# omahs/celestia-app

Measured on AMD Instinct MI355X. Metric: EDS+DAH squares/sec (k=128), higher is better.
Workload: dtype u8; 1 GPU; k=128 ODS -> EDS + 4k NMT roots + DAH, batch replay; k=128, field=GF(2^8), parallelism=batch1, input_layout=ODS in Q0 of the EDS buffer (placed by the upload), batches_in_flight=4

## Files before the change

celestia-app_amd/csrc/nmt_device.hpp:

```cpp
#pragma once
#include <hip/hip_runtime.h>

#include "cel_internal.hpp"
#include "sha256_device.hpp"

namespace cel {

__device__ __forceinline__ void load_node(const uint32_t* p, uint32_t (&n)[kNodeWords]) {
  const uint4* q = reinterpret_cast<const uint4*>(p);
#pragma unroll
  for (int i = 0; i < 6; i++) {
    const uint4 v = q[i];
    n[4 * i] = v.x; n[4 * i + 1] = v.y; n[4 * i + 2] = v.z; n[4 * i + 3] = v.w;
  }
}

__device__ __forceinline__ void store_node(uint32_t* p, const uint32_t (&n)[kNodeWords]) {
  uint4* q = reinterpret_cast<uint4*>(p);
#pragma unroll
  for (int i = 0; i < 6; i++) q[i] = make_uint4(n[4 * i], n[4 * i + 1], n[4 * i + 2], n[4 * i + 3]);
}

__device__ __forceinline__ void put_digest(uint32_t (&nd)[kNodeWords], const uint32_t (&st)[8]) {
  uint32_t sw[8];
#pragma unroll
  for (int i = 0; i < 8; i++) sw[i] = bswap32(st[i]);
  nd[14] = (nd[14] & 0xFFFFu) | (sw[0] << 16);
#pragma unroll
  for (int i = 15; i <= 21; i++) nd[i] = __builtin_amdgcn_alignbyte(sw[i - 14], sw[i - 15], 2);
  nd[22] = sw[7] >> 16;
  nd[23] = 0;
}


constexpr uint32_t kLeafParPrefix[7] = {0x00FFFFFFu, 0xFFFFFFFFu, 0xFFFFFFFFu, 0xFFFFFFFFu,
                                        0xFFFFFFFFu, 0xFFFFFFFFu, 0xFFFFFFFFu};
constexpr ShaMid kLeafParMid = sha_midstate(kLeafParPrefix, 7);

template <bool PF>
__device__ __forceinline__ void leaf_hash(uint32_t (&st)[8], const uint32_t* __restrict__ sh, bool q0) {
  sha256_init(st);
  uint32_t w[16];
  uint32_t nx[17];
  auto load17 = [&](int b) {
    const uint32_t* base = sh + 16 * b - 8;
    const uint4* p4 = reinterpret_cast<const uint4*>(base);
#pragma unroll
    for (int i = 0; i < 4; i++) {
      const uint4 v = p4[i];
      nx[4 * i] = v.x; nx[4 * i + 1] = v.y; nx[4 * i + 2] = v.z; nx[4 * i + 3] = v.w;
    }
    nx[16] = base[16];
  };
  {
    uint32_t s[9];
    const uint4* p4 = reinterpret_cast<const uint4*>(sh);
    const uint4 v0 = p4[0], v1 = p4[1];
    s[0] = v0.x; s[1] = v0.y; s[2] = v0.z; s[3] = v0.w; s[4] = v1.x; s[5] = v1.y; s[6] = v1.z; s[7] = v1.w;
    s[8] = sh[8];
    if (PF) load17(1);
#pragma unroll
    for (int i = 8; i < 16; i++) w[i] = perm(s[i - 8], s[i - 7], 0x06070001u);
    if (__all(!q0)) {
#pragma unroll
      for (int i = 0; i < 7; i++) w[i] = kLeafParPrefix[i];
      w[7] = 0xFFFF0000u | perm(0u, s[0], 0x0C0C0001u);
      sha256_compress_from<7>(st, mid_regs(kLeafParMid), w);
    } else {
      if (q0) {
        w[0] = perm(0u, s[0], 0x0C000102u);
#pragma unroll
        for (int i = 1; i < 7; i++) w[i] = perm(s[i - 1], s[i], 0x07000102u);
        w[7] = perm(s[6], s[7], 0x07000C0Cu) | perm(0u, s[0], 0x0C0C0001u);
      } else {
#pragma unroll
        for (int i = 0; i < 7; i++) w[i] = kLeafParPrefix[i];
        w[7] = 0xFFFF0000u | perm(0u, s[0], 0x0C0C0001u);
      }
      sha256_compress(st, w);
    }
  }
#pragma unroll 1
  for (int b = 1; b < 8; b++) {
    if (!PF) load17(b);
#pragma unroll
    for (int i = 0; i < 16; i++) w[i] = perm(nx[i], nx[i + 1], 0x06070001u);
    if (PF) {
      if (b < 7) {
        load17(b + 1);
      } else {
        const uint4* p4 = reinterpret_cast<const uint4*>(sh + 120);
        const uint4 v0 = p4[0], v1 = p4[1];
        nx[0] = v0.x; nx[1] = v0.y; nx[2] = v0.z; nx[3] = v0.w; nx[4] = v1.x; nx[5] = v1.y; nx[6] = v1.z; nx[7] = v1.w;
      }
    }
    sha256_compress(st, w);
  }
  {
    if (!PF) {
      const uint4* p4 = reinterpret_cast<const uint4*>(sh + 120);
      const uint4 v0 = p4[0], v1 = p4[1];
      nx[0] = v0.x; nx[1] = v0.y; nx[2] = v0.z; nx[3] = v0.w; nx[4] = v1.x; nx[5] = v1.y; nx[6] = v1.z; nx[7] = v1.w;
    }
#pragma unroll
    for (int i = 0; i < 7; i++) w[i] = perm(nx[i], nx[i + 1], 0x06070001u);
    w[7] = perm(nx[7], 0x80u, 0x0607000Cu);
#pragma unroll
    for (int i = 8; i < 15; i++) w[i] = 0u;
    w[15] = 542u * 8u;
    sha256_compress(st, w);
  }
}

__device__ __forceinline__ void leaf_record(const uint32_t* __restrict__ sh, bool q0, const uint32_t (&st)[8],
                                            uint32_t (&nd)[kNodeWords]) {
  if (q0) {
    const uint4* p4 = reinterpret_cast<const uint4*>(sh);
    uint32_t s[8];
    const uint4 v0 = p4[0], v1 = p4[1];
    s[0] = v0.x; s[1] = v0.y; s[2] = v0.z; s[3] = v0.w; s[4] = v1.x; s[5] = v1.y; s[6] = v1.z; s[7] = v1.w;
#pragma unroll
    for (int i = 0; i < 7; i++) nd[i] = s[i];
    nd[7] = (s[7] & 0xFFu) | (s[0] << 8);
#pragma unroll
    for (int i = 0; i < 6; i++) nd[8 + i] = __builtin_amdgcn_alignbyte(s[i + 1], s[i], 3);
    nd[14] = (s[6] >> 24) | ((s[7] & 0xFFu) << 8);
  } else {
#pragma unroll
    for (int i = 0; i < 14; i++) nd[i] = 0xFFFFFFFFu;
    nd[14] = 0xFFFFu;
  }
  put_digest(nd, st);
}

template <bool PF>
__device__ __forceinline__ void make_leaf_node(const uint32_t* __restrict__ sh, bool q0, uint32_t (&nd)[kNodeWords]) {
  uint32_t st[8];
  leaf_hash<PF>(st, sh, q0);
  leaf_record(sh, q0, st, nd);
}

__device__ __forceinline__ bool ns_less(const uint32_t* __restrict__ a, const uint32_t* __restrict__ b) {
  const uint4* pa = reinterpret_cast<const uint4*>(a);
  const uint4* pb = reinterpret_cast<const uint4*>(b);
  uint32_t x[8], y[8];
#pragma unroll
  for (int i = 0; i < 2; i++) {
    const uint4 u = pa[i], v = pb[i];
    x[4 * i] = u.x; x[4 * i + 1] = u.y; x[4 * i + 2] = u.z; x[4 * i + 3] = u.w;
    y[4 * i] = v.x; y[4 * i + 1] = v.y; y[4 * i + 2] = v.z; y[4 * i + 3] = v.w;
  }
  int res = 0;
#pragma unroll
  for (int i = 0; i < 8; i++) {
    uint32_t xa = bswap32(x[i]), yb = bswap32(y[i]);
    if (i == 7) { xa &= 0xFF000000u; yb &= 0xFF000000u; }
    if (res == 0 && xa != yb) res = xa < yb ? -1 : 1;
  }
  return res < 0;
}

__device__ __forceinline__ bool min_is_parity(const uint32_t* __restrict__ R) {
  bool par = (R[7] & 0xFFu) == 0xFFu;
#pragma unroll
  for (int q = 0; q < 7; q++) par = par && (R[q] == 0xFFFFFFFFu);
  return par;
}


constexpr uint32_t kNodeParPrefix[14] = {0x01FFFFFFu, 0xFFFFFFFFu, 0xFFFFFFFFu, 0xFFFFFFFFu, 0xFFFFFFFFu,
                                         0xFFFFFFFFu, 0xFFFFFFFFu, 0xFFFFFFFFu, 0xFFFFFFFFu, 0xFFFFFFFFu,
                                         0xFFFFFFFFu, 0xFFFFFFFFu, 0xFFFFFFFFu, 0xFFFFFFFFu};
constexpr ShaMid kNodeParMid = sha_midstate(kNodeParPrefix, 14);

__device__ __forceinline__ uint32_t node_word(const uint32_t (&L)[kNodeWords], const uint32_t (&R)[kNodeWords], int q) {
  if (q == 0) return perm(1u, L[0], 0x04000102u);
  if (q <= 21) return perm(L[q - 1], L[q], 0x07000102u);
  if (q == 22) return perm(L[21], L[22], 0x0700010Cu) | (R[0] & 0xFFu);
  if (q <= 44) return perm(R[q - 23], R[q - 22], 0x05060700u);
  if (q == 45) return perm(R[22], 0x80u, 0x05000C0Cu);
  if (q == 47) return 181u * 8u;
  return 0u;
}

__device__ __forceinline__ void hash_node(const uint32_t (&L)[kNodeWords], const uint32_t (&R)[kNodeWords],
                                          uint32_t (&out)[kNodeWords]) {
  uint32_t st[8];
  sha256_init(st);
  bool lpar = (L[14] & 0xFFFFu) == 0xFFFFu;
#pragma unroll
  for (int i = 0; i < 14; i++) lpar = lpar && (L[i] == 0xFFFFFFFFu);
  {
    uint32_t w[16];
    if (__all(lpar)) {
#pragma unroll
      for (int wi = 0; wi < 14; wi++) w[wi] = kNodeParPrefix[wi];
      w[14] = node_word(L, R, 14);
      w[15] = node_word(L, R, 15);
      sha256_compress_from<14>(st, mid_regs(kNodeParMid), w);
    } else {
#pragma unroll
      for (int wi = 0; wi < 16; wi++) w[wi] = node_word(L, R, wi);
      sha256_compress(st, w);
    }
  }
#pragma unroll
  for (int b = 1; b < 3; b++) {
    uint32_t w[16];
#pragma unroll
    for (int wi = 0; wi < 16; wi++) w[wi] = node_word(L, R, 16 * b + wi);
    sha256_compress(st, w);
  }
  bool rpar = (R[7] & 0xFFu) == 0xFFu;
#pragma unroll
  for (int i = 0; i < 7; i++) rpar = rpar && (R[i] == 0xFFFFFFFFu);
#pragma unroll
  for (int i = 0; i < 7; i++) out[i] = L[i];
  const uint32_t X7 = rpar ? L[7] : R[7];
  out[7] = (L[7] & 0xFFu) | (X7 & 0xFFFFFF00u);
#pragma unroll
  for (int i = 8; i < 14; i++) out[i] = rpar ? L[i] : R[i];
  out[14] = (rpar ? L[14] : R[14]) & 0xFFFFu;
  put_digest(out, st);
}

__device__ __forceinline__ void hash_pair(const uint32_t* in, uint64_t li, uint64_t ri, uint32_t (&o)[kNodeWords]) {
  uint32_t L[kNodeWords], R[kNodeWords];
  load_node(in + li * kNodeWords, L);
  load_node(in + ri * kNodeWords, R);
  hash_node(L, R, o);
}


__device__ __forceinline__ void sha_empty(uint32_t (&st)[8]) {
  uint32_t w[16];
  w[0] = 0x80000000u;
#pragma unroll
  for (int i = 1; i < 16; i++) w[i] = 0;
  sha256_init(st);
  sha256_compress(st, w);
}

__device__ __forceinline__ void rfc_leaf90(const uint32_t (&R)[kNodeWords], uint32_t (&st)[8]) {
  sha256_init(st);
#pragma unroll
  for (int b = 0; b < 2; b++) {
    uint32_t w[16];
#pragma unroll
    for (int wi = 0; wi < 16; wi++) {
      const int q = 16 * b + wi;
      uint32_t x;
      if (q == 0) x = perm(0u, R[0], 0x0C000102u);
      else if (q <= 21) x = perm(R[q - 1], R[q], 0x07000102u);
      else if (q == 22) x = perm(R[21], R[22], 0x0700010Cu) | 0x80u;
      else if (q == 31) x = 91u * 8u;
      else x = 0u;
      w[wi] = x;
    }
    sha256_compress(st, w);
  }
}

__device__ __forceinline__ void rfc_inner(const uint32_t* l, const uint32_t* r, uint32_t (&st)[8]) {
  uint32_t w[16];
  w[0] = 0x01000000u | (l[0] >> 8);
#pragma unroll
  for (int i = 1; i < 8; i++) w[i] = __builtin_amdgcn_alignbit(l[i - 1], l[i], 8);
  w[8] = __builtin_amdgcn_alignbit(l[7], r[0], 8);
#pragma unroll
  for (int i = 9; i < 16; i++) w[i] = __builtin_amdgcn_alignbit(r[i - 9], r[i - 8], 8);
  sha256_init(st);
  uint32_t w2[16];
  w2[0] = (r[7] << 24) | 0x00800000u;
#pragma unroll
  for (int i = 1; i < 15; i++) w2[i] = 0;
  w2[15] = 65u * 8u;
  sha256_compress(st, w);
  sha256_compress(st, w2);
}

}
```

celestia-app_amd/csrc/nmt_kernels.hip:

```cpp
#include <hip/hip_runtime.h>

#include <climits>

#include "cel_internal.hpp"
#include "nmt_device.hpp"
#include "nmt_host.hpp"
#include "sha256_device.hpp"

namespace cel {




template <bool ORDER, bool PF>
__global__ __launch_bounds__(256) void k_leaf(const uint8_t* __restrict__ eds, uint32_t k, uint32_t* __restrict__ leaves,
                                              int32_t* __restrict__ bad_axis, uint32_t cell0, uint32_t cell1) {
  const uint32_t W = 2 * k;
  const uint32_t cell = cell0 + blockIdx.x * 256u + threadIdx.x;
  if (cell >= cell1) return;
  const uint32_t r = cell / W, c = cell % W;
  const uint64_t sq_eds = (uint64_t)W * W * kShare;
  const uint32_t* sh = reinterpret_cast<const uint32_t*>(eds + blockIdx.y * sq_eds + (uint64_t)cell * kShare);
  const bool q0 = (r < k) && (c < k);
  {
    uint32_t nd[kNodeWords];
    make_leaf_node<PF>(sh, q0, nd);
    store_node(leaves + ((uint64_t)blockIdx.y * W * W + cell) * kNodeWords, nd);
  }
  __builtin_amdgcn_sched_barrier(0);
  if (ORDER && q0) {
    if (c > 0 && ns_less(sh, sh - kShare / 4)) atomicMin(bad_axis + blockIdx.y, (int32_t)r);
    if (r > 0 && ns_less(sh, sh - (uint64_t)W * kShare / 4)) atomicMin(bad_axis + blockIdx.y, (int32_t)(W + c));
  }
}


__device__ __forceinline__ void put_root(const uint32_t (&o)[kNodeWords], uint32_t sq, uint32_t t, uint32_t W,
                                         uint32_t* __restrict__ leafd, uint8_t* __restrict__ row_out,
                                         uint8_t* __restrict__ col_out) {
  {
    uint8_t* r = (t < W ? row_out + ((uint64_t)sq * W + t) * kNode : col_out + ((uint64_t)sq * W + (t - W)) * kNode);
    uint16_t* r16 = reinterpret_cast<uint16_t*>(r);
#pragma unroll
    for (int i = 0; i < 45; i++) r16[i] = (uint16_t)(o[i / 2] >> (16 * (i & 1)));
  }
  if (leafd) {
    uint32_t st[8];
    rfc_leaf90(o, st);
    uint4* d = reinterpret_cast<uint4*>(leafd + ((uint64_t)sq * 2 * W + t) * 8);
    d[0] = make_uint4(st[0], st[1], st[2], st[3]);
    d[1] = make_uint4(st[4], st[5], st[6], st[7]);
  }
}

template <bool FROM_LEAVES>
__global__ __launch_bounds__(256) void k_level(const uint32_t* __restrict__ in, uint32_t* __restrict__ out, uint32_t W,
                                               uint32_t nin, uint32_t trees, uint32_t* __restrict__ leafd,
                                               uint8_t* __restrict__ row_out, uint8_t* __restrict__ col_out) {
  const uint32_t nout = nin / 2;
  const uint32_t idx = blockIdx.x * 256u + threadIdx.x;
  if (idx >= trees * nout) return;
  const uint32_t t = idx / nout, j = idx % nout;
  uint64_t li, ri;
  if (FROM_LEAVES) {
    const uint64_t sq = (uint64_t)blockIdx.y * W * W;
    if (t < W) { li = sq + (uint64_t)t * W + 2 * j; ri = li + 1; }
    else { li = sq + (uint64_t)(2 * j) * W + (t - W); ri = li + W; }
  } else {
    const uint64_t sq = (uint64_t)blockIdx.y * trees * nin;
    li = sq + (uint64_t)t * nin + 2 * j;
    ri = li + 1;
  }
  uint32_t o[kNodeWords];
  hash_pair(in, li, ri, o);
  const uint64_t oi = (uint64_t)blockIdx.y * trees * nout + idx;
  store_node(out + oi * kNodeWords, o);
  if (row_out) put_root(o, blockIdx.y, t, W, leafd, row_out, col_out);
}


template <bool ORDER, bool PF, bool ROOTS>
__global__ __launch_bounds__(256) __attribute__((amdgpu_waves_per_eu(3, 3))) void k_leaf_quad(
    const uint8_t* __restrict__ eds, uint32_t k, uint32_t* __restrict__ out, int32_t* __restrict__ bad_axis,
    uint32_t* __restrict__ leafd, uint8_t* __restrict__ row_out, uint8_t* __restrict__ col_out) {
  const uint32_t W = 2 * k, trees = 2 * W;
  const uint32_t tw = k < 8 ? k : 8u, th = 64 / tw, tiles_x = k / tw;
  const uint32_t g = blockIdx.x * 256u + threadIdx.x, tile = g / 64, l = g % 64;
  const uint32_t bi = (tile / tiles_x) * th + l / tw, bj = (tile % tiles_x) * tw + l % tw;
  if (bi >= k) return;
  const uint64_t sq_eds = (uint64_t)W * W * kShare;
  const uint32_t* sh00 =
      reinterpret_cast<const uint32_t*>(eds + blockIdx.y * sq_eds + ((uint64_t)(2 * bi) * W + 2 * bj) * kShare);
  uint32_t dA[8], dB[8], dC[8];
#pragma unroll 1
  for (uint32_t s = 0; s < 4; s++) {
    const uint32_t r = 2 * bi + (s >> 1), c = 2 * bj + (s & 1);
    const uint32_t* sh = sh00 + ((uint64_t)(s >> 1) * W + (s & 1)) * (kShare / 4);
    const bool q0 = (r < k) && (c < k);
    {
      uint32_t st[8];
      leaf_hash<PF>(st, sh, q0);
#pragma unroll
      for (int i = 0; i < 8; i++) {
        if (s == 0 || s == 3) dA[i] = st[i];
        if (s == 1) dB[i] = st[i];
        if (s == 2) dC[i] = st[i];
      }
    }
    const uint32_t nn = s == 3 ? 2u : (s ? 1u : 0u);
#pragma unroll 1
    for (uint32_t n = 0; n < nn; n++) {
      const uint32_t lc = s < 3 ? 0u : 1u + n;
      const bool row = (s == 1) || (s == 3 && n == 1);
      const uint32_t* shl = sh00 + ((uint64_t)(lc >> 1) * W + (lc & 1)) * (kShare / 4);
      const bool q0l = (2 * bi + (lc >> 1) < k) && (2 * bj + (lc & 1) < k);
      uint32_t o[kNodeWords];
      {
        uint32_t L[kNodeWords], R[kNodeWords], dl[8], dr[8];
#pragma unroll
        for (int i = 0; i < 8; i++) {
          dl[i] = lc == 0 ? dA[i] : (lc == 1 ? dB[i] : dC[i]);
          dr[i] = s == 1 ? dB[i] : (s == 2 ? dC[i] : dA[i]);
        }
        leaf_record(shl, q0l, dl, L);
        leaf_record(sh, q0, dr, R);
        hash_node(L, R, o);
      }
      const uint32_t t = row ? r : W + c, idx = row ? bj : bi;
      store_node(out + (((uint64_t)blockIdx.y * trees + t) * k + idx) * kNodeWords, o);
      if (ROOTS) put_root(o, blockIdx.y, t, W, leafd, row_out, col_out);
    }
    __builtin_amdgcn_sched_barrier(0);
    if (ORDER && q0) {
      if (c > 0 && ns_less(sh, sh - kShare / 4)) atomicMin(bad_axis + blockIdx.y, (int32_t)r);
      if (r > 0 && ns_less(sh, sh - (uint64_t)W * kShare / 4)) atomicMin(bad_axis + blockIdx.y, (int32_t)(W + c));
    }
  }
}



__global__ __launch_bounds__(1024) void k_merkle(const uint32_t* __restrict__ items, const uint32_t* __restrict__ leafd,
                                                uint32_t n, uint8_t* dah, const int32_t* __restrict__ bad_axis,
                                                int32_t* status, const uint8_t* out_src,
                                                uint8_t* __restrict__ host_out, uint32_t out_bytes) {
  extern __shared__ __attribute__((aligned(16))) uint32_t hs[];
  const uint32_t g = blockIdx.x;
  const uint32_t* it = items + (uint64_t)g * n * kNodeWords;
  if (leafd) {
    for (uint32_t i = threadIdx.x; i < n * 8; i += blockDim.x) hs[i] = leafd[(uint64_t)g * n * 8 + i];
  } else {
    for (uint32_t i = threadIdx.x; i < n; i += blockDim.x) {
      uint32_t R[kNodeWords], st[8];
      load_node(it + (uint64_t)i * kNodeWords, R);
      rfc_leaf90(R, st);
#pragma unroll
      for (int j = 0; j < 8; j++) hs[i * 8 + j] = st[j];
    }
  }
  __syncthreads();
  uint32_t cnt = n;
  while (cnt > 1) {
    const uint32_t half = cnt / 2;
    uint32_t st[8];
    for (uint32_t base = 0; base < half; base += blockDim.x) {
      const uint32_t i = base + threadIdx.x;
      if (i < half) rfc_inner(hs + (2 * i) * 8, hs + (2 * i + 1) * 8, st);
      __syncthreads();
      if (i < half) {
#pragma unroll
        for (int j = 0; j < 8; j++) hs[i * 8 + j] = st[j];
      }
      __syncthreads();
    }
    if (cnt & 1) {
      if (threadIdx.x < 8) hs[half * 8 + threadIdx.x] = hs[(cnt - 1) * 8 + threadIdx.x];
      __syncthreads();
    }
    cnt = half + (cnt & 1);
  }
  if (threadIdx.x == 0) {
    uint32_t st[8];
    if (n == 0) sha_empty(st);
    else
      for (int j = 0; j < 8; j++) st[j] = hs[j];
    for (int j = 0; j < 8; j++) {
      dah[g * 32 + 4 * j] = (uint8_t)(st[j] >> 24);
      dah[g * 32 + 4 * j + 1] = (uint8_t)(st[j] >> 16);
      dah[g * 32 + 4 * j + 2] = (uint8_t)(st[j] >> 8);
      dah[g * 32 + 4 * j + 3] = (uint8_t)st[j];
    }
    if (status) status[g] = (bad_axis && bad_axis[g] != INT_MAX) ? CEL_EORDER : CEL_OK;
  }
  if (host_out) {
    __threadfence();
    __syncthreads();
    const uint4* src = reinterpret_cast<const uint4*>(out_src);
    uint4* dst = reinterpret_cast<uint4*>(host_out);
    for (uint32_t i = threadIdx.x; i < out_bytes / 16; i += blockDim.x) dst[i] = src[i];
  }
}

static uint32_t merkle_block(uint32_t n) {
  const uint32_t pairs = ((n / 2 + 63) / 64) * 64;
  return pairs < 64 ? 64u : (pairs > 1024 ? 1024u : pairs);
}

__global__ __launch_bounds__(256) void k_dah_leaves(const uint32_t* __restrict__ items, uint32_t n,
                                                    uint32_t* __restrict__ leafd, uint8_t* __restrict__ row_out,
                                                    uint8_t* __restrict__ col_out) {
  const uint32_t i = blockIdx.x * 256u + threadIdx.x;
  if (i >= n) return;
  uint32_t R[kNodeWords], st[8];
  load_node(items + (uint64_t)i * kNodeWords, R);
  rfc_leaf90(R, st);
  uint4* d = reinterpret_cast<uint4*>(leafd + (uint64_t)i * 8);
  d[0] = make_uint4(st[0], st[1], st[2], st[3]);
  d[1] = make_uint4(st[4], st[5], st[6], st[7]);
  const uint32_t half = n / 2;
  uint16_t* r16 = reinterpret_cast<uint16_t*>(i < half ? row_out + (uint64_t)i * kNode : col_out + (uint64_t)(i - half) * kNode);
#pragma unroll
  for (int j = 0; j < 45; j++) r16[j] = (uint16_t)(R[j / 2] >> (16 * (j & 1)));
}

__global__ void k_fill_i32(int32_t* p, uint32_t n, int32_t v) {
  const uint32_t i = blockIdx.x * blockDim.x + threadIdx.x;
  if (i < n) p[i] = v;
}


void launch_fill_i32(int32_t* p, uint32_t n, int32_t v, uint32_t block, hipStream_t s) {
  hipLaunchKernelGGL(k_fill_i32, dim3((n + block - 1) / block), dim3(block), 0, s, p, n, v);
}

void launch_dah_leaves(const uint32_t* items, uint32_t n, uint32_t* leafd, uint8_t* row_out, uint8_t* col_out,
                       hipStream_t s) {
  hipLaunchKernelGGL(k_dah_leaves, dim3((n + 255) / 256), dim3(256), 0, s, items, n, leafd, row_out, col_out);
}

void launch_merkle(const uint32_t* items, const uint32_t* leafd, uint32_t n, uint32_t lists, uint8_t* dah,
                   const int32_t* bad_axis, int32_t* status, hipStream_t s, const uint8_t* out_src, uint8_t* host_out,
                   uint32_t out_bytes) {
  const size_t lds = (size_t)(n ? n : 1) * 8 * 4;
  hipLaunchKernelGGL(k_merkle, dim3(lists), dim3(merkle_block(n)), lds, s, items, leafd, n, dah, bad_axis, status,
                     out_src, host_out, out_bytes);
}

struct CommitWork {
  uint32_t *leaves, *ping, *pong, *roots, *leafd;
  int32_t* bad;
  size_t size;
};

static bool quad_path(uint32_t nsq) { return nsq > 1; }

static CommitWork commit_work(void* work, uint32_t k, uint32_t nsq) {
  const size_t W = 2 * (size_t)k, nb = kNodeWords * 4;
  Carver c(work);
  CommitWork w;
  w.leaves = c.take<uint32_t>(quad_path(nsq) ? 0 : nsq * W * W * nb);
  w.ping = c.take<uint32_t>(nsq * 2 * W * (W / 2 + 1) * nb);
  w.pong = c.take<uint32_t>(nsq * 2 * W * (W / 4 + 1) * nb);
  w.roots = c.take<uint32_t>(nsq * 2 * W * nb);
  w.bad = c.take<int32_t>((size_t)nsq * 4 + 4);
  w.leafd = c.take<uint32_t>(nsq * 2 * W * 32);
  w.size = c.size();
  return w;
}

size_t nmt_workspace_size(uint32_t k, uint32_t nsq) { return commit_work(nullptr, k, nsq).size; }

hipError_t launch_commit_leaves(const uint8_t* eds, uint32_t k, uint32_t nsq, void* work, bool order_check,
                                uint32_t row0, uint32_t row1, bool init_bad, hipStream_t s) {
  if (quad_path(nsq)) return hipErrorInvalidValue;
  const uint32_t W = 2 * k;
  const CommitWork w = commit_work(work, k, nsq);
  const Range r("nmt.leaf");
  if (init_bad) launch_fill_i32(w.bad, nsq, INT_MAX, 256, s);
  const uint32_t c0 = row0 * W, c1 = row1 * W;
  if (c1 <= c0) return hipGetLastError();
  dim3 gl((c1 - c0 + 255) / 256, nsq);
  dispatch_order_pf(order_check, latency_bound((uint64_t)(c1 - c0) * nsq), [&](auto order, auto pf) {
    hipLaunchKernelGGL((k_leaf<decltype(order)::value, decltype(pf)::value>), gl, dim3(256), 0, s, eds, k, w.leaves,
                       w.bad, c0, c1);
  });
  return hipGetLastError();
}

static hipError_t commit_levels(const CommitWork& w, bool from_leaves, uint32_t k, uint32_t nsq, uint8_t* row_roots,
                                uint8_t* col_roots, uint8_t* dah, int32_t* status, hipStream_t s, uint8_t* host_out,
                                uint32_t out_bytes) {
  const uint32_t W = 2 * k;
  const uint32_t trees = 2 * W;
  uint32_t nin = from_leaves ? W : W / 2;
  const uint32_t* src = from_leaves ? w.leaves : w.ping;
  uint32_t* dst = from_leaves ? w.ping : w.pong;
  bool first = from_leaves;
  roctxRangePushA("nmt.levels");
  while (nin > 1) {
    const uint32_t nout = nin / 2;
    uint32_t* out = (nout == 1) ? w.roots : dst;
    uint32_t* ld = (nout == 1 && dah) ? w.leafd : nullptr;
    dim3 g((trees * nout + 255) / 256, nsq);
    uint8_t* ro = (nout == 1) ? row_roots : nullptr;
    uint8_t* co = (nout == 1) ? col_roots : nullptr;
    if (first) hipLaunchKernelGGL(k_level<true>, g, dim3(256), 0, s, src, out, W, nin, trees, ld, ro, co);
    else hipLaunchKernelGGL(k_level<false>, g, dim3(256), 0, s, src, out, W, nin, trees, ld, ro, co);
    first = false;
    src = out;
    dst = (dst == w.ping) ? w.pong : w.ping;
    nin = nout;
  }
  roctxRangePop();
  const Range r("dah");
  if (dah)
    launch_merkle(w.roots, w.leafd, trees, nsq, dah, w.bad, status, s, host_out ? row_roots : nullptr, host_out,
                  out_bytes);
  return hipGetLastError();
}

hipError_t launch_commit_trees(uint32_t k, uint32_t nsq, uint8_t* row_roots, uint8_t* col_roots, uint8_t* dah,
                               int32_t* status, void* work, hipStream_t s, uint8_t* host_out, uint32_t out_bytes) {
  if (quad_path(nsq)) return hipErrorInvalidValue;
  return commit_levels(commit_work(work, k, nsq), true, k, nsq, row_roots, col_roots, dah, status, s, host_out,
                       out_bytes);
}

static hipError_t launch_commit_quads(const uint8_t* eds, uint32_t k, uint32_t nsq, const CommitWork& w,
                                      bool order_check, uint8_t* row_roots, uint8_t* col_roots, bool want_dah,
                                      hipStream_t s) {
  const Range r("nmt.leaf");
  launch_fill_i32(w.bad, nsq, INT_MAX, 256, s);
  const uint32_t tw = k < 8 ? k : 8u, th = 64 / tw;
  const uint64_t lanes = (uint64_t)((k + th - 1) / th) * (k / tw) * 64;
  dim3 g((uint32_t)((lanes + 255) / 256), nsq);
  if (k == 1) {
    uint32_t* ld = want_dah ? w.leafd : nullptr;
    if (order_check)
      hipLaunchKernelGGL((k_leaf_quad<true, false, true>), g, dim3(256), 0, s, eds, k, w.roots, w.bad, ld,
                         row_roots, col_roots);
    else
      hipLaunchKernelGGL((k_leaf_quad<false, false, true>), g, dim3(256), 0, s, eds, k, w.roots, w.bad, ld,
                         row_roots, col_roots);
    return hipGetLastError();
  }
  dispatch_order_pf(order_check, latency_bound(lanes * nsq), [&](auto order, auto pf) {
    hipLaunchKernelGGL((k_leaf_quad<decltype(order)::value, decltype(pf)::value, false>), g, dim3(256), 0, s, eds, k,
                       w.ping, w.bad, nullptr, nullptr, nullptr);
  });
  return hipGetLastError();
}

hipError_t launch_commit(const uint8_t* eds, uint32_t k, uint32_t nsq, uint8_t* row_roots, uint8_t* col_roots,
                         uint8_t* dah, int32_t* status, void* work, bool order_check, hipStream_t s) {
  if (!quad_path(nsq)) {
    hipError_t e = launch_commit_leaves(eds, k, nsq, work, order_check, 0, 2 * k, true, s);
    if (e == hipSuccess) e = launch_commit_trees(k, nsq, row_roots, col_roots, dah, status, work, s);
    return e;
  }
  const CommitWork w = commit_work(work, k, nsq);
  hipError_t e = launch_commit_quads(eds, k, nsq, w, order_check, row_roots, col_roots, dah != nullptr, s);
  if (e == hipSuccess) e = commit_levels(w, false, k, nsq, row_roots, col_roots, dah, status, s, nullptr, 0);
  return e;
}


}
```

celestia-app_amd/csrc/sha256_device.hpp:

```cpp
#pragma once
#include <hip/hip_runtime.h>

#include <cstdint>

namespace cel {

__device__ __forceinline__ uint32_t rotr32(uint32_t x, uint32_t n) { return __builtin_amdgcn_alignbit(x, x, n); }
__device__ __forceinline__ uint32_t xor3(uint32_t a, uint32_t b, uint32_t c) {
  return __builtin_amdgcn_bitop3_b32(a, b, c, 0x96);
}
__device__ __forceinline__ uint32_t maj3(uint32_t a, uint32_t b, uint32_t c) {
  return __builtin_amdgcn_bitop3_b32(a, b, c, 0xE8);
}

__device__ __forceinline__ uint32_t bswap32(uint32_t x) { return __builtin_amdgcn_perm(0u, x, 0x00010203u); }

struct Sha256 {
  uint32_t h[8];
  __device__ __forceinline__ void init() {
    h[0] = 0x6a09e667u; h[1] = 0xbb67ae85u; h[2] = 0x3c6ef372u; h[3] = 0xa54ff53au;
    h[4] = 0x510e527fu; h[5] = 0x9b05688cu; h[6] = 0x1f83d9abu; h[7] = 0x5be0cd19u;
  }
};

__constant__ const uint32_t kSha256K[64] = {
    0x428a2f98u, 0x71374491u, 0xb5c0fbcfu, 0xe9b5dba5u, 0x3956c25bu, 0x59f111f1u, 0x923f82a4u, 0xab1c5ed5u,
    0xd807aa98u, 0x12835b01u, 0x243185beu, 0x550c7dc3u, 0x72be5d74u, 0x80deb1feu, 0x9bdc06a7u, 0xc19bf174u,
    0xe49b69c1u, 0xefbe4786u, 0x0fc19dc6u, 0x240ca1ccu, 0x2de92c6fu, 0x4a7484aau, 0x5cb0a9dcu, 0x76f988dau,
    0x983e5152u, 0xa831c66du, 0xb00327c8u, 0xbf597fc7u, 0xc6e00bf3u, 0xd5a79147u, 0x06ca6351u, 0x14292967u,
    0x27b70a85u, 0x2e1b2138u, 0x4d2c6dfcu, 0x53380d13u, 0x650a7354u, 0x766a0abbu, 0x81c2c92eu, 0x92722c85u,
    0xa2bfe8a1u, 0xa81a664bu, 0xc24b8b70u, 0xc76c51a3u, 0xd192e819u, 0xd6990624u, 0xf40e3585u, 0x106aa070u,
    0x19a4c116u, 0x1e376c08u, 0x2748774cu, 0x34b0bcb5u, 0x391c0cb3u, 0x4ed8aa4au, 0x5b9cca4fu, 0x682e6ff3u,
    0x748f82eeu, 0x78a5636fu, 0x84c87814u, 0x8cc70208u, 0x90befffau, 0xa4506cebu, 0xbef9a3f7u, 0xc67178f2u};

struct ShaRegs {
  uint32_t a, b, c, d, e, f, g, h;
};

__device__ __forceinline__ void sha_round(ShaRegs& r, uint32_t kw) {
  const uint32_t S1 = xor3(rotr32(r.e, 6), rotr32(r.e, 11), rotr32(r.e, 25));
  const uint32_t ch = (r.e & r.f) | (~r.e & r.g);
  const uint32_t t1 = r.h + S1 + ch + kw;
  const uint32_t S0 = xor3(rotr32(r.a, 2), rotr32(r.a, 13), rotr32(r.a, 22));
  const uint32_t t2 = S0 + maj3(r.a, r.b, r.c);
  r.h = r.g; r.g = r.f; r.f = r.e; r.e = r.d + t1; r.d = r.c; r.c = r.b; r.b = r.a; r.a = t1 + t2;
}

template <int START>
__device__ __forceinline__ void sha256_compress_from(uint32_t (&st)[8], const ShaRegs& r0, uint32_t (&w)[16]) {
  ShaRegs r = r0;
#pragma unroll
  for (int i = START; i < 16; i++) sha_round(r, w[i] + kSha256K[i]);
#pragma unroll 1
  for (int base = 16; base < 64; base += 16) {
#pragma unroll
    for (int j = 0; j < 16; j++) {
      const uint32_t w15 = w[(j + 1) & 15], w2 = w[(j + 14) & 15];
      const uint32_t s0 = xor3(rotr32(w15, 7), rotr32(w15, 18), w15 >> 3);
      const uint32_t s1 = xor3(rotr32(w2, 17), rotr32(w2, 19), w2 >> 10);
      const uint32_t wi = w[j] + s0 + w[(j + 9) & 15] + s1;
      w[j] = wi;
      sha_round(r, wi + kSha256K[base + j]);
    }
  }
  st[0] += r.a; st[1] += r.b; st[2] += r.c; st[3] += r.d;
  st[4] += r.e; st[5] += r.f; st[6] += r.g; st[7] += r.h;
}

__device__ __forceinline__ void sha256_compress(uint32_t (&st)[8], uint32_t (&w)[16]) {
  sha256_compress_from<0>(st, ShaRegs{st[0], st[1], st[2], st[3], st[4], st[5], st[6], st[7]}, w);
}

__device__ __forceinline__ void sha256_compress_unrolled(uint32_t (&st)[8], uint32_t (&w)[16]) {
  ShaRegs r{st[0], st[1], st[2], st[3], st[4], st[5], st[6], st[7]};
#pragma unroll
  for (int i = 0; i < 16; i++) sha_round(r, w[i] + kSha256K[i]);
#pragma unroll
  for (int i = 16; i < 64; i++) {
    const int j = i & 15;
    const uint32_t w15 = w[(j + 1) & 15], w2 = w[(j + 14) & 15];
    const uint32_t s0 = xor3(rotr32(w15, 7), rotr32(w15, 18), w15 >> 3);
    const uint32_t s1 = xor3(rotr32(w2, 17), rotr32(w2, 19), w2 >> 10);
    const uint32_t wi = w[j] + s0 + w[(j + 9) & 15] + s1;
    w[j] = wi;
    sha_round(r, wi + kSha256K[i]);
  }
  st[0] += r.a; st[1] += r.b; st[2] += r.c; st[3] += r.d;
  st[4] += r.e; st[5] += r.f; st[6] += r.g; st[7] += r.h;
}

struct ShaMid {
  uint32_t v[8];
};
constexpr uint32_t kShaKc[64] = {
    0x428a2f98u, 0x71374491u, 0xb5c0fbcfu, 0xe9b5dba5u, 0x3956c25bu, 0x59f111f1u, 0x923f82a4u, 0xab1c5ed5u,
    0xd807aa98u, 0x12835b01u, 0x243185beu, 0x550c7dc3u, 0x72be5d74u, 0x80deb1feu, 0x9bdc06a7u, 0xc19bf174u};
constexpr uint32_t c_rotr(uint32_t x, int n) { return (x >> n) | (x << (32 - n)); }
constexpr ShaMid sha_midstate(const uint32_t* w, int n) {
  uint32_t a = 0x6a09e667u, b = 0xbb67ae85u, c = 0x3c6ef372u, d = 0xa54ff53au;
  uint32_t e = 0x510e527fu, f = 0x9b05688cu, g = 0x1f83d9abu, h = 0x5be0cd19u;
  for (int i = 0; i < n; i++) {
    const uint32_t t1 = h + (c_rotr(e, 6) ^ c_rotr(e, 11) ^ c_rotr(e, 25)) + ((e & f) ^ (~e & g)) + kShaKc[i] + w[i];
    const uint32_t t2 = (c_rotr(a, 2) ^ c_rotr(a, 13) ^ c_rotr(a, 22)) + ((a & b) ^ (a & c) ^ (b & c));
    h = g; g = f; f = e; e = d + t1; d = c; c = b; b = a; a = t1 + t2;
  }
  return ShaMid{{a, b, c, d, e, f, g, h}};
}
__device__ __forceinline__ ShaRegs mid_regs(const ShaMid& m) {
  return ShaRegs{m.v[0], m.v[1], m.v[2], m.v[3], m.v[4], m.v[5], m.v[6], m.v[7]};
}

__device__ __forceinline__ void sha256_init(uint32_t (&st)[8]) {
  st[0] = 0x6a09e667u; st[1] = 0xbb67ae85u; st[2] = 0x3c6ef372u; st[3] = 0xa54ff53au;
  st[4] = 0x510e527fu; st[5] = 0x9b05688cu; st[6] = 0x1f83d9abu; st[7] = 0x5be0cd19u;
}

__device__ __forceinline__ uint32_t perm(uint32_t s0, uint32_t s1, uint32_t sel) {
  return __builtin_amdgcn_perm(s0, s1, sel);
}

}
```

Before: 22780 squares/s.

## Split NMT levels into Q0 and parity trees with constant-folded parity hashing

Nodes whose subtree lies entirely in parity shares have a fixed max-namespace prefix. They are now stored as bare 32-byte digests in a separate buffer and hashed with a specialized SHA-256 that uses precomputed constant message words, a midstate and constant folding. Original-data (Q0) nodes keep the full node path. The level kernels process both kinds in one launch and the root level rebuilds full parity records. This cuts memory traffic and SHA work for three quarters of the tree nodes, at the cost of more complex indexing and new constants (kNodeParMid) whose correctness must match the reference.

```diff
diff --git a/celestia-app_amd/csrc/nmt_device.hpp b/celestia-app_amd/csrc/nmt_device.hpp
--- a/celestia-app_amd/csrc/nmt_device.hpp
+++ b/celestia-app_amd/csrc/nmt_device.hpp
@@ -232,6 +232,80 @@
 }
 
 
+constexpr uint32_t kParNodeWords[48] = {
+    0x01FFFFFFu, 0xFFFFFFFFu, 0xFFFFFFFFu, 0xFFFFFFFFu, 0xFFFFFFFFu, 0xFFFFFFFFu, 0xFFFFFFFFu, 0xFFFFFFFFu,
+    0xFFFFFFFFu, 0xFFFFFFFFu, 0xFFFFFFFFu, 0xFFFFFFFFu, 0xFFFFFFFFu, 0xFFFFFFFFu, 0xFFFFFF00u, 0x00000000u,
+    0x00000000u, 0x00000000u, 0x00000000u, 0x00000000u, 0x00000000u, 0x00000000u, 0x000000FFu, 0xFFFFFFFFu,
+    0xFFFFFFFFu, 0xFFFFFFFFu, 0xFFFFFFFFu, 0xFFFFFFFFu, 0xFFFFFFFFu, 0xFFFFFFFFu, 0xFFFFFFFFu, 0xFFFFFFFFu,
+    0xFFFFFFFFu, 0xFFFFFFFFu, 0xFFFFFFFFu, 0xFFFFFFFFu, 0xFFFFFFFFu, 0xFF000000u, 0x00000000u, 0x00000000u,
+    0x00000000u, 0x00000000u, 0x00000000u, 0x00000000u, 0x00000000u, 0x00800000u, 0x00000000u, 181u * 8u};
+
+template <bool COMPACT>
+__device__ __forceinline__ void hash_parity_node(const uint32_t (&dl)[8], const uint32_t (&dr)[8],
+                                                 uint32_t (&out)[8]) {
+  constexpr int kEnd = COMPACT ? 32 : 64;
+  uint32_t st[8], w[16];
+  sha256_init(st);
+  auto finish = [&](ShaRegs& r) {
+    if (COMPACT) sha256_rounds_tail(r, w);
+    sha256_add(st, r);
+  };
+  {
+#pragma unroll
+    for (int i = 0; i < 14; i++) w[i] = kParNodeWords[i];
+    w[14] = kParNodeWords[14] | (dl[0] >> 24);
+    w[15] = __builtin_amdgcn_alignbit(dl[0], dl[1], 24);
+    ShaRegs r = mid_regs(kNodeParMid);
+    sha256_rounds_folded<14, kEnd>(r, w);
+    finish(r);
+  }
+  {
+#pragma unroll
+    for (int i = 0; i < 6; i++) w[i] = __builtin_amdgcn_alignbit(dl[i + 1], dl[i + 2], 24);
+    w[6] = kParNodeWords[22] | (dl[7] << 8);
+#pragma unroll
+    for (int i = 7; i < 16; i++) w[i] = kParNodeWords[16 + i];
+    ShaRegs r{st[0], st[1], st[2], st[3], st[4], st[5], st[6], st[7]};
+    sha256_rounds_folded<0, kEnd>(r, w);
+    finish(r);
+  }
+  {
+#pragma unroll
+    for (int i = 0; i < 5; i++) w[i] = kParNodeWords[32 + i];
+    w[5] = kParNodeWords[37] | (dr[0] >> 8);
+#pragma unroll
+    for (int i = 6; i < 13; i++) w[i] = __builtin_amdgcn_alignbit(dr[i - 6], dr[i - 5], 8);
+    w[13] = kParNodeWords[45] | (dr[7] << 24);
+    w[14] = kParNodeWords[46];
+    w[15] = kParNodeWords[47];
+    ShaRegs r{st[0], st[1], st[2], st[3], st[4], st[5], st[6], st[7]};
+    sha256_rounds_folded<0, kEnd>(r, w);
+    finish(r);
+  }
+#pragma unroll
+  for (int i = 0; i < 8; i++) out[i] = st[i];
+}
+
+__device__ __forceinline__ void parity_record(const uint32_t (&d)[8], uint32_t (&nd)[kNodeWords]) {
+#pragma unroll
+  for (int i = 0; i < 14; i++) nd[i] = 0xFFFFFFFFu;
+  nd[14] = 0xFFFFu;
+  put_digest(nd, d);
+}
+
+__device__ __forceinline__ void load_digest(const uint32_t* p, uint32_t (&d)[8]) {
+  const uint4* q = reinterpret_cast<const uint4*>(p);
+  const uint4 a = q[0], b = q[1];
+  d[0] = a.x; d[1] = a.y; d[2] = a.z; d[3] = a.w; d[4] = b.x; d[5] = b.y; d[6] = b.z; d[7] = b.w;
+}
+
+__device__ __forceinline__ void store_digest(uint32_t* p, const uint32_t (&d)[8]) {
+  uint4* q = reinterpret_cast<uint4*>(p);
+  q[0] = make_uint4(d[0], d[1], d[2], d[3]);
+  q[1] = make_uint4(d[4], d[5], d[6], d[7]);
+}
+
+
 __device__ __forceinline__ void sha_empty(uint32_t (&st)[8]) {
   uint32_t w[16];
   w[0] = 0x80000000u;
diff --git a/celestia-app_amd/csrc/nmt_kernels.hip b/celestia-app_amd/csrc/nmt_kernels.hip
--- a/celestia-app_amd/csrc/nmt_kernels.hip
+++ b/celestia-app_amd/csrc/nmt_kernels.hip
@@ -79,10 +79,63 @@
 }
 
 
+__host__ __device__ constexpr uint32_t q_nodes(uint32_t k, uint32_t n) { return k * n; }
+__host__ __device__ constexpr uint32_t p_nodes(uint32_t k, uint32_t n) { return 3 * k * n; }
+__device__ __forceinline__ uint32_t q_node(uint32_t k, uint32_t n, uint32_t t, uint32_t i) {
+  return (t < k ? t : t - k) * (n / 2) + i;
+}
+__device__ __forceinline__ uint32_t p_node(uint32_t k, uint32_t n, uint32_t t, uint32_t i) {
+  const uint32_t W = 2 * k, a = t < W ? t : t - W;
+  if (a < k) return (t < W ? a : k + a) * (n / 2) + (i - n / 2);
+  return k * n + (t < W ? a - k : a) * n + i;
+}
+
+template <bool ROOT>
+__global__ __launch_bounds__(256) void k_level_split(const uint32_t* __restrict__ qin, uint32_t* __restrict__ qout,
+                                                     const uint32_t* __restrict__ pin, uint32_t* __restrict__ pout,
+                                                     uint32_t nq, uint32_t np, uint32_t bq, uint32_t k,
+                                                     uint32_t* __restrict__ leafd, uint8_t* __restrict__ row_out,
+                                                     uint8_t* __restrict__ col_out) {
+  const uint32_t sq = blockIdx.y, W = 2 * k;
+  if (blockIdx.x < bq) {
+    const uint32_t i = blockIdx.x * 256u + threadIdx.x;
+    if (i >= nq) return;
+    uint32_t o[kNodeWords];
+    if (ROOT) {
+      uint32_t L[kNodeWords], R[kNodeWords], d[8];
+      load_node(qin + ((uint64_t)sq * nq + i) * kNodeWords, L);
+      load_digest(pin + ((uint64_t)sq * 3 * np + i) * 8, d);
+      parity_record(d, R);
+      hash_node(L, R, o);
+      put_root(o, sq, i < k ? i : W + (i - k), W, leafd, row_out, col_out);
+    } else {
+      hash_pair(qin + (uint64_t)sq * 2 * nq * kNodeWords, 2 * i, 2 * i + 1, o);
+      store_node(qout + ((uint64_t)sq * nq + i) * kNodeWords, o);
+    }
+  } else {
+    const uint32_t i = (blockIdx.x - bq) * 256u + threadIdx.x;
+    if (i >= np) return;
+    const uint32_t* in = pin + (ROOT ? (uint64_t)sq * 3 * np + np : (uint64_t)sq * 2 * np) * 8;
+    uint32_t dl[8], dr[8], d[8];
+    load_digest(in + (uint64_t)i * 16, dl);
+    load_digest(in + (uint64_t)i * 16 + 8, dr);
+    hash_parity_node<false>(dl, dr, d);
+    if (ROOT) {
+      uint32_t o[kNodeWords];
+      parity_record(d, o);
+      put_root(o, sq, i < k ? k + i : W + i, W, leafd, row_out, col_out);
+    } else {
+      store_digest(pout + ((uint64_t)sq * np + i) * 8, d);
+    }
+  }
+}
+
+
 template <bool ORDER, bool PF, bool ROOTS>
 __global__ __launch_bounds__(256) __attribute__((amdgpu_waves_per_eu(3, 3))) void k_leaf_quad(
-    const uint8_t* __restrict__ eds, uint32_t k, uint32_t* __restrict__ out, int32_t* __restrict__ bad_axis,
-    uint32_t* __restrict__ leafd, uint8_t* __restrict__ row_out, uint8_t* __restrict__ col_out) {
+    const uint8_t* __restrict__ eds, uint32_t k, uint32_t* __restrict__ out, uint32_t* __restrict__ pout,
+    int32_t* __restrict__ bad_axis, uint32_t* __restrict__ leafd, uint8_t* __restrict__ row_out,
+    uint8_t* __restrict__ col_out) {
   const uint32_t W = 2 * k, trees = 2 * W;
   const uint32_t tw = k < 8 ? k : 8u, th = 64 / tw, tiles_x = k / tw;
   const uint32_t g = blockIdx.x * 256u + threadIdx.x, tile = g / 64, l = g % 64;
@@ -114,21 +167,35 @@
       const bool row = (s == 1) || (s == 3 && n == 1);
       const uint32_t* shl = sh00 + ((uint64_t)(lc >> 1) * W + (lc & 1)) * (kShare / 4);
       const bool q0l = (2 * bi + (lc >> 1) < k) && (2 * bj + (lc & 1) < k);
-      uint32_t o[kNodeWords];
-      {
-        uint32_t L[kNodeWords], R[kNodeWords], dl[8], dr[8];
+      const uint32_t t = row ? r : W + c, idx = row ? bj : bi;
+      auto children = [&](uint32_t (&dl)[8], uint32_t (&dr)[8]) {
 #pragma unroll
         for (int i = 0; i < 8; i++) {
           dl[i] = lc == 0 ? dA[i] : (lc == 1 ? dB[i] : dC[i]);
           dr[i] = s == 1 ? dB[i] : (s == 2 ? dC[i] : dA[i]);
         }
-        leaf_record(shl, q0l, dl, L);
-        leaf_record(sh, q0, dr, R);
-        hash_node(L, R, o);
+      };
+      if (ROOTS || q0l) {
+        uint32_t o[kNodeWords];
+        {
+          uint32_t L[kNodeWords], R[kNodeWords], dl[8], dr[8];
+          children(dl, dr);
+          leaf_record(shl, q0l, dl, L);
+          leaf_record(sh, q0, dr, R);
+          hash_node(L, R, o);
+        }
+        if (ROOTS) {
+          store_node(out + (((uint64_t)blockIdx.y * trees + t) * k + idx) * kNodeWords, o);
+          put_root(o, blockIdx.y, t, W, leafd, row_out, col_out);
+        } else {
+          store_node(out + ((uint64_t)blockIdx.y * q_nodes(k, k) + q_node(k, k, t, idx)) * kNodeWords, o);
+        }
+      } else {
+        uint32_t dl[8], dr[8], o[8];
+        children(dl, dr);
+        hash_parity_node<true>(dl, dr, o);
+        store_digest(pout + ((uint64_t)blockIdx.y * p_nodes(k, k) + p_node(k, k, t, idx)) * 8, o);
       }
-      const uint32_t t = row ? r : W + c, idx = row ? bj : bi;
-      store_node(out + (((uint64_t)blockIdx.y * trees + t) * k + idx) * kNodeWords, o);
-      if (ROOTS) put_root(o, blockIdx.y, t, W, leafd, row_out, col_out);
     }
     __builtin_amdgcn_sched_barrier(0);
     if (ORDER && q0) {
@@ -248,6 +315,7 @@
 
 struct CommitWork {
   uint32_t *leaves, *ping, *pong, *roots, *leafd;
+  uint32_t *q[2], *p[2];
   int32_t* bad;
   size_t size;
 };
@@ -265,6 +333,11 @@
   w.bad = c.take<int32_t>((size_t)nsq * 4 + 4);
   w.leafd = c.take<uint32_t>(nsq * 2 * W * 32);
   w.size = c.size();
+  for (uint32_t i = 0; i < 2; i++) {
+    Carver a(i ? w.pong : w.ping);
+    w.q[i] = a.take<uint32_t>((size_t)nsq * q_nodes(k, k >> i) * nb);
+    w.p[i] = a.take<uint32_t>((size_t)nsq * p_nodes(k, k >> i) * 32);
+  }
   return w;
 }
 
@@ -287,15 +360,24 @@
   return hipGetLastError();
 }
 
-static hipError_t commit_levels(const CommitWork& w, bool from_leaves, uint32_t k, uint32_t nsq, uint8_t* row_roots,
+static hipError_t commit_dah(const CommitWork& w, uint32_t k, uint32_t nsq, uint8_t* row_roots, uint8_t* dah,
+                             int32_t* status, hipStream_t s, uint8_t* host_out, uint32_t out_bytes) {
+  const Range r("dah");
+  if (dah)
+    launch_merkle(w.roots, w.leafd, 4 * k, nsq, dah, w.bad, status, s, host_out ? row_roots : nullptr, host_out,
+                  out_bytes);
+  return hipGetLastError();
+}
+
+static hipError_t commit_levels(const CommitWork& w, uint32_t k, uint32_t nsq, uint8_t* row_roots,
                                 uint8_t* col_roots, uint8_t* dah, int32_t* status, hipStream_t s, uint8_t* host_out,
                                 uint32_t out_bytes) {
   const uint32_t W = 2 * k;
   const uint32_t trees = 2 * W;
-  uint32_t nin = from_leaves ? W : W / 2;
-  const uint32_t* src = from_leaves ? w.leaves : w.ping;
-  uint32_t* dst = from_leaves ? w.ping : w.pong;
-  bool first = from_leaves;
+  uint32_t nin = W;
+  const uint32_t* src = w.leaves;
+  uint32_t* dst = w.ping;
+  bool first = true;
   roctxRangePushA("nmt.levels");
   while (nin > 1) {
     const uint32_t nout = nin / 2;
@@ -312,18 +394,13 @@
     nin = nout;
   }
   roctxRangePop();
-  const Range r("dah");
-  if (dah)
-    launch_merkle(w.roots, w.leafd, trees, nsq, dah, w.bad, status, s, host_out ? row_roots : nullptr, host_out,
-                  out_bytes);
-  return hipGetLastError();
+  return commit_dah(w, k, nsq, row_roots, dah, status, s, host_out, out_bytes);
 }
 
 hipError_t launch_commit_trees(uint32_t k, uint32_t nsq, uint8_t* row_roots, uint8_t* col_roots, uint8_t* dah,
                                int32_t* status, void* work, hipStream_t s, uint8_t* host_out, uint32_t out_bytes) {
   if (quad_path(nsq)) return hipErrorInvalidValue;
-  return commit_levels(commit_work(work, k, nsq), true, k, nsq, row_roots, col_roots, dah, status, s, host_out,
-                       out_bytes);
+  return commit_levels(commit_work(work, k, nsq), k, nsq, row_roots, col_roots, dah, status, s, host_out, out_bytes);
 }
 
 static hipError_t launch_commit_quads(const uint8_t* eds, uint32_t k, uint32_t nsq, const CommitWork& w,
@@ -337,17 +414,32 @@
   if (k == 1) {
     uint32_t* ld = want_dah ? w.leafd : nullptr;
     if (order_check)
-      hipLaunchKernelGGL((k_leaf_quad<true, false, true>), g, dim3(256), 0, s, eds, k, w.roots, w.bad, ld,
+      hipLaunchKernelGGL((k_leaf_quad<true, false, true>), g, dim3(256), 0, s, eds, k, w.roots, nullptr, w.bad, ld,
                          row_roots, col_roots);
     else
-      hipLaunchKernelGGL((k_leaf_quad<false, false, true>), g, dim3(256), 0, s, eds, k, w.roots, w.bad, ld,
+      hipLaunchKernelGGL((k_leaf_quad<false, false, true>), g, dim3(256), 0, s, eds, k, w.roots, nullptr, w.bad, ld,
                          row_roots, col_roots);
     return hipGetLastError();
   }
   dispatch_order_pf(order_check, latency_bound(lanes * nsq), [&](auto order, auto pf) {
     hipLaunchKernelGGL((k_leaf_quad<decltype(order)::value, decltype(pf)::value, false>), g, dim3(256), 0, s, eds, k,
-                       w.ping, w.bad, nullptr, nullptr, nullptr);
+                       w.q[0], w.p[0], w.bad, nullptr, nullptr, nullptr);
   });
+  return hipGetLastError();
+}
+
+static hipError_t commit_levels_split(const CommitWork& w, uint32_t k, uint32_t nsq, uint8_t* row_roots,
+                                      uint8_t* col_roots, bool want_dah, hipStream_t s) {
+  const Range r("nmt.levels");
+  uint32_t at = 0;
+  for (uint32_t n = k; n > 2; n /= 2, at ^= 1) {
+    const uint32_t nq = q_nodes(k, n / 2), np = p_nodes(k, n / 2), bq = (nq + 255) / 256;
+    hipLaunchKernelGGL(k_level_split<false>, dim3(bq + (np + 255) / 256, nsq), dim3(256), 0, s, w.q[at], w.q[at ^ 1],
+                       w.p[at], w.p[at ^ 1], nq, np, bq, k, nullptr, nullptr, nullptr);
+  }
+  const uint32_t nr = 2 * k, bq = (nr + 255) / 256;
+  hipLaunchKernelGGL(k_level_split<true>, dim3(2 * bq, nsq), dim3(256), 0, s, w.q[at], nullptr, w.p[at], nullptr, nr,
+                     nr, bq, k, want_dah ? w.leafd : nullptr, row_roots, col_roots);
   return hipGetLastError();
 }
 
@@ -360,7 +452,8 @@
   }
   const CommitWork w = commit_work(work, k, nsq);
   hipError_t e = launch_commit_quads(eds, k, nsq, w, order_check, row_roots, col_roots, dah != nullptr, s);
-  if (e == hipSuccess) e = commit_levels(w, false, k, nsq, row_roots, col_roots, dah, status, s, nullptr, 0);
+  if (e == hipSuccess && k > 1) e = commit_levels_split(w, k, nsq, row_roots, col_roots, dah != nullptr, s);
+  if (e == hipSuccess) e = commit_dah(w, k, nsq, row_roots, dah, status, s, nullptr, 0);
   return e;
 }
 
diff --git a/celestia-app_amd/csrc/sha256_device.hpp b/celestia-app_amd/csrc/sha256_device.hpp
--- a/celestia-app_amd/csrc/sha256_device.hpp
+++ b/celestia-app_amd/csrc/sha256_device.hpp
@@ -11,6 +11,17 @@
 }
 __device__ __forceinline__ uint32_t maj3(uint32_t a, uint32_t b, uint32_t c) {
   return __builtin_amdgcn_bitop3_b32(a, b, c, 0xE8);
+}
+template <bool FOLD>
+__device__ __forceinline__ uint32_t xor3f(uint32_t a, uint32_t b, uint32_t c) {
+  if (FOLD && __builtin_constant_p(a) && __builtin_constant_p(b) && __builtin_constant_p(c)) return a ^ b ^ c;
+  return xor3(a, b, c);
+}
+template <bool FOLD>
+__device__ __forceinline__ uint32_t maj3f(uint32_t a, uint32_t b, uint32_t c) {
+  if (FOLD && __builtin_constant_p(a) && __builtin_constant_p(b) && __builtin_constant_p(c))
+    return (a & b) | (a & c) | (b & c);
+  return maj3(a, b, c);
 }
 
 __device__ __forceinline__ uint32_t bswap32(uint32_t x) { return __builtin_amdgcn_perm(0u, x, 0x00010203u); }
@@ -37,12 +48,13 @@
   uint32_t a, b, c, d, e, f, g, h;
 };
 
+template <bool FOLD = false>
 __device__ __forceinline__ void sha_round(ShaRegs& r, uint32_t kw) {
-  const uint32_t S1 = xor3(rotr32(r.e, 6), rotr32(r.e, 11), rotr32(r.e, 25));
+  const uint32_t S1 = xor3f<FOLD>(rotr32(r.e, 6), rotr32(r.e, 11), rotr32(r.e, 25));
   const uint32_t ch = (r.e & r.f) | (~r.e & r.g);
   const uint32_t t1 = r.h + S1 + ch + kw;
-  const uint32_t S0 = xor3(rotr32(r.a, 2), rotr32(r.a, 13), rotr32(r.a, 22));
-  const uint32_t t2 = S0 + maj3(r.a, r.b, r.c);
+  const uint32_t S0 = xor3f<FOLD>(rotr32(r.a, 2), rotr32(r.a, 13), rotr32(r.a, 22));
+  const uint32_t t2 = S0 + maj3f<FOLD>(r.a, r.b, r.c);
   r.h = r.g; r.g = r.f; r.f = r.e; r.e = r.d + t1; r.d = r.c; r.c = r.b; r.b = r.a; r.a = t1 + t2;
 }
 
@@ -89,6 +101,43 @@
   st[4] += r.e; st[5] += r.f; st[6] += r.g; st[7] += r.h;
 }
 
+template <int START, int END>
+__device__ __forceinline__ void sha256_rounds_folded(ShaRegs& r, uint32_t (&w)[16]) {
+#pragma unroll
+  for (int i = START; i < 16; i++) sha_round<true>(r, w[i] + kSha256K[i]);
+#pragma unroll
+  for (int i = 16; i < END; i++) {
+    const int j = i & 15;
+    const uint32_t w15 = w[(j + 1) & 15], w2 = w[(j + 14) & 15];
+    const uint32_t s0 = xor3f<true>(rotr32(w15, 7), rotr32(w15, 18), w15 >> 3);
+    const uint32_t s1 = xor3f<true>(rotr32(w2, 17), rotr32(w2, 19), w2 >> 10);
+    uint32_t wi = w[j] + s0 + w[(j + 9) & 15] + s1;
+    if (!__builtin_constant_p(wi)) asm volatile("" : "+v"(wi), "+v"(r.e));
+    w[j] = wi;
+    sha_round<true>(r, wi + kSha256K[i]);
+  }
+}
+
+__device__ __forceinline__ void sha256_add(uint32_t (&st)[8], const ShaRegs& r) {
+  st[0] += r.a; st[1] += r.b; st[2] += r.c; st[3] += r.d;
+  st[4] += r.e; st[5] += r.f; st[6] += r.g; st[7] += r.h;
+}
+
+__device__ __forceinline__ void sha256_rounds_tail(ShaRegs& r, uint32_t (&w)[16]) {
+#pragma unroll 1
+  for (int base = 32; base < 64; base += 16) {
+#pragma unroll
+    for (int j = 0; j < 16; j++) {
+      const uint32_t w15 = w[(j + 1) & 15], w2 = w[(j + 14) & 15];
+      const uint32_t s0 = xor3(rotr32(w15, 7), rotr32(w15, 18), w15 >> 3);
+      const uint32_t s1 = xor3(rotr32(w2, 17), rotr32(w2, 19), w2 >> 10);
+      const uint32_t wi = w[j] + s0 + w[(j + 9) & 15] + s1;
+      w[j] = wi;
+      sha_round(r, wi + kSha256K[base + j]);
+    }
+  }
+}
+
 struct ShaMid {
   uint32_t v[8];
 };
```

Result: faster. 23140 squares/s (median of 6 runs) (+1.6%).
